# iamgroot42/A-LINK

Hardware: AMD Instinct MI355X
Metric: 112x112 face embeddings/sec (IR-ResNet-100 ArcFace, 512-d, L2-normalised) (higher is better)
Workload: dtype bf16

## Files before the change

a-link_amd/csrc/alink_common.h:

```cpp
#pragma once
#include <hip/hip_runtime.h>
#include <stdint.h>
#include <stddef.h>
#include <string>

#include "../../include/alink_hip.h"
#include "conv_kernel.h"

namespace alink {

void set_error(const char* fmt, ...);
int  hip_fail(hipError_t e, const char* what, const char* file, int line);

#define ALINK_HIP(call)                                                          \
    do {                                                                         \
        hipError_t e__ = (call);                                                 \
        if (e__ != hipSuccess) return ::alink::hip_fail(e__, #call, __FILE__, __LINE__); \
    } while (0)

#define ALINK_REQUIRE(cond, code, ...)          \
    do {                                        \
        if (!(cond)) {                          \
            ::alink::set_error(__VA_ARGS__);    \
            return (code);                      \
// ... 78 lines not shown
    const float* slabs;
    const float* bias;
    float*       out;
    float*       norms;
    int S, M, E;
    float scale;
    int*  nonfinite;
};
hipError_t launch_fc_finish(const FcFinishParams& p, hipStream_t stream);
hipError_t launch_absmax_f16(const void* x, size_t n_elements, unsigned* out_bits, hipStream_t stream);
hipError_t launch_conv_split_finish(int dtype, const ConvParams& p, const float* slabs, int S, hipStream_t stream);

ConvKernel direct_variant(int ksz, int stride, int pad, int H, int W, int Cin, int Cout);
ConvKernel direct_variant_tiles(int ksz, int stride, int pad, int H, int W, int Cin, int Cout);
ConvKernel linear_variant_x2(int ksz, int stride, int pad, int H, int W, int Cin, int Cout);
hipError_t launch_conv(ConvKernel k, int dtype, const ConvParams& p, hipStream_t st);
hipError_t direct_set_attributes();
ConvKernel linear_variant(int ksz, int stride, int pad, int H, int W, int Cin, int Cout);
ConvKernel c64_variant(int ksz, int stride, int pad, int H, int W, int Cin, int Cout);
ConvKernel s2c64_variant(int ksz, int stride, int pad, int H, int W, int Cin, int Cout);
hipError_t launch_conv3x3_linear(ConvKernel k, int dtype, const ConvParams& p, hipStream_t st);
hipError_t launch_conv3x3_c64(int dtype, const ConvParams& p, hipStream_t st);
hipError_t launch_conv3x3_s2c64(int dtype, const ConvParams& p, hipStream_t st);
hipError_t c64_set_attributes();
hipError_t s2c64_set_attributes();
hipError_t linear_set_attributes();
hipError_t linear_check_contract();
bool       front_c64_applies(int dtype, int H, int W, int C0, int Cout);
hipError_t front_c64_set_attributes();
hipError_t launch_front_c64(int dtype, const ConvParams& conv1, const StemParams& stem, void* xs, bool slopes_le_1, hipStream_t st);
bool       unit_c64_applies(int dtype, const ConvParams& c1, const ConvParams& c2);
hipError_t unit_c64_set_attributes();
hipError_t launch_unit_c64(int dtype, const ConvParams& c1, const ConvParams& c2, hipStream_t st);
bool       conv3x3_lat_applies(int dtype, const ConvParams& p);
hipError_t launch_conv3x3_lat(int dtype, const ConvParams& p, hipStream_t stream);
bool       conv_gemm_lat_applies(int dtype, const ConvParams& p);
hipError_t launch_conv_gemm_lat(int dtype, const ConvParams& p, hipStream_t stream);

hipError_t launch_l2norm_bwd(int dtype, const float* g, const float* e, const float* norms, void* dz, int M, int E,
                             hipStream_t st);
hipError_t launch_zero_insert(int dtype, const void* in, void* out, int N, int H, int W, int Ho, int Wo, int C,
                              hipStream_t st);
hipError_t launch_stem_bwd(int dtype, const void* dy0, const void* y0, const float* w, const float* alpha, float* dpix,
                           int N, int H, int W, float mul, int nchw, hipStream_t st);

hipError_t launch_r50_grad_scale(const float* dfeat, int count, int HW, float* scale, hipStream_t st);
hipError_t launch_r50_avgpool_bwd(int dtype, const float* dfeat, const void* y, void* dz, const float* scale, int N, int HW, int C,
                                  hipStream_t st);
hipError_t launch_r50_relu_mask(int dtype, void* g, const void* y, long long count, hipStream_t st);
hipError_t launch_r50_scatter_mask(int dtype, const void* in, const void* y, void* out, int N, int H, int W, int Ho, int Wo, int C,
                                   hipStream_t st);
hipError_t launch_r50_maxpool_bwd(int dtype, const void* y0, const void* pooled, const void* g, void* d0, int N, int H, int W, int C,
                                  int Hp, int Wp, hipStream_t st);
hipError_t launch_r50_stem_bwd(int dtype, const void* d0, const void* wfrag, float* dpix, const float* scale, int N, int H, int W,
                               int Ho, int Wo, int pad_t, int pad_l, int flip, hipStream_t st);
int r50_stem_bwd_max_width();

uint16_t f32_to_bf16_rne(float f);
uint16_t f32_to_f16_rne(float f);

int init_kernels();

__device__ __forceinline__ float relu_keep_nan(float v) { return v < 0.f ? 0.f : v; }
__device__ __forceinline__ float max_keep_nan(float a, float b) { return (a < b || b != b) ? b : a; }

}
// ... 13 lines not shown
```

a-link_amd/csrc/backbone.hip:

```cpp
#include "alink_common.h"

#include <algorithm>
#include <cmath>
#include <cstdarg>
#include <cstdio>
#include <cstring>
#include <map>
#include <string>
#include <vector>

namespace alink {

static thread_local char g_err[1024] = "";
void set_error(const char* fmt, ...) {
    va_list ap;
    va_start(ap, fmt);
    vsnprintf(g_err, sizeof(g_err), fmt, ap);
    va_end(ap);
}
int hip_fail(hipError_t e, const char* what, const char* file, int line) {
    set_error("HIP error %d (%s) in `%s` at %s:%d", (int)e, hipGetErrorString(e), what, file, line);
    return ALINK_EHIP;
}

// ... 660 lines not shown
    if (!traits(k).fine) return 0;
    const int sib = (g_sibling_aware && k != ConvKernel::Linear7) ? siblings : 1;
    return linear_grid(M, Cout, 128) * sib <= g_fine_max ? 1 : 0;
}
int g_ablate = 0;
int g_stop_after = 0;
extern "C" void alink_debug_set_stop_after(int n) { g_stop_after = n; }
int g_stagger = 0;
int g_shard_stagger = 0;
extern "C" void alink_debug_set_shard_stagger(int on) { g_shard_stagger = on; }

int g_fuse_unit = 1;
constexpr int FUSE_UNIT_MIN_N = 64;
extern "C" void alink_debug_set_fuse_unit(int mode) { g_fuse_unit = mode; }
extern "C" void alink_debug_set_stagger(int n) { g_stagger = n < 0 ? 0 : n; }
void* g_stamps = nullptr;
int g_prof_reps = 4;
extern "C" void alink_debug_set_profile_reps(int n) { g_prof_reps = n < 1 ? 1 : n; }
extern "C" void alink_debug_set_ablate(int a) { g_ablate = a; }
extern "C" void alink_debug_set_stamps(void* p) { g_stamps = p; }

static const ConvLayer* fusable_unit(const alink_backbone* bb, const ConvLayer& L, int N, int S, bool cache) {
    if (!g_fuse_unit || (g_fuse_unit == 1 && N < FUSE_UNIT_MIN_N) || cache || S != 1 || g_ablate || g_stamps) return nullptr;
    const int dt = bb->cfg.dtype;
    if (dt != ALINK_DT_BF16 && dt != ALINK_DT_F16) return nullptr;
    const size_t i = (size_t)(&L - bb->convs.data());
    if (L.role != 1 || i + 1 >= bb->convs.size()) return nullptr;
    const ConvLayer& L2 = bb->convs[i + 1];
    if (L2.role != 3 || L2.unit != L.unit || L2.Cin2 || L2.in_buf != L.out_buf || L2.resid_buf != L.in_buf) return nullptr;
    if (L.kernel != ConvKernel::Linear56 || L2.kernel != ConvKernel::Linear56 || L.stride != 1 || L2.stride != 1) return nullptr;
    if (L.Cin != 64 || L.Cout != 64 || L2.Cin != 64 || L2.Cout != 64 || L.Hin != 56 || L.Win != 56) return nullptr;
    if (plan_split(bb, L2, N) != 1) return nullptr;
    return &L2;
}

static int embed_impl(alink_backbone_t* bb, const void* dev_in, int layout, int N, float* dev_out,
                      void* ws, size_t ws_bytes, hipStream_t stream, float* ms, double* flops, int* kind,
                      int* n_launches, const GradLayout* cache = nullptr, int calib = 0, hipEvent_t front_done = nullptr) {
    ALINK_REQUIRE(bb && dev_in && dev_out && ws, ALINK_EINVAL, "NULL argument");
    ALINK_REQUIRE(bb->finalized, ALINK_ESTATE, "alink_embed before alink_backbone_finalize");
    ALINK_REQUIRE(N > 0, ALINK_EINVAL, "n_images must be positive");
    ALINK_REQUIRE(layout >= 0 && layout <= 2, ALINK_EINVAL, "unknown pixel layout %d", layout);
    const alink_ir_cfg& cfg = bb->cfg;
    ALINK_REQUIRE((long long)N * cfg.height * cfg.width * 64 * (cfg.dtype == ALINK_DT_F16X2 ? 2 : 1) < (1ll << 31), ALINK_EINVAL,
                  "batch of %d images exceeds the 2^31-element activation limit; split the batch", N);
    size_t off[7], total;
    ws_layout(bb, N, off, &total);
    if (cache) total = cache->total;
    ALINK_REQUIRE(ws_bytes >= total, ALINK_ENOMEM, "workspace too small: %zu < %zu", ws_bytes, total);
    ALINK_REQUIRE(((uintptr_t)ws & 255) == 0, ALINK_EINVAL, "workspace must be 256-byte aligned");
    char* base = (char*)ws;
    auto buf = [&](int id) -> void* { return base + off[id]; };

    const bool prof = ms != nullptr;
    const int reps = prof ? g_prof_reps : 1;
    const int cap = prof ? *n_launches : 0;
    int nl = 0;
    std::vector<hipEvent_t> ev;
    std::vector<int> split_pairs;
    auto mark = [&]() -> int {
        if (!prof) return ALINK_OK;
        hipEvent_t e;
        ALINK_HIP(hipEventCreate(&e));
        ALINK_HIP(hipEventRecord(e, stream));
        ev.push_back(e);
        return ALINK_OK;
// ... 102 lines not shown
                    ConvParams q = p;
                    if (S > 1) {
                        q.out = buf(6); q.splitk = S; q.ksteps_per_split = p.ksteps_per_split / S;
                    }
                    ALINK_HIP(launch_conv(L.kernel, cfg.dtype, q, stream));
                    if (S > 1) ALINK_HIP(launch_conv_split_finish(cfg.dtype, p, (const float*)buf(6), S, stream));
                }
                return ALINK_OK;
            });
            if (rc) return rc;
            bexp[L.out_buf] = L.e_out;
        } else if (front && &L == &bb->convs[0]) {
            p.stamps = g_stamps;
            for (int r = 0; r < reps; ++r) ALINK_HIP(launch_front_c64(cfg.dtype, p, sp, buf(0), bb->front_slopes_le_1, stream));
            note(conv_flops(p) + 2.0 * N * cfg.height * cfg.width * 64.0 * 27.0, 1);
            if ((rc = mark())) return rc;
            last_out = L.out_buf;
            continue;
        } else if (const ConvLayer* L2 = fusable_unit(bb, L, N, S, cache != nullptr)) {
            ConvParams p2 = p;
            p2.in = buf(L2->in_buf); p2.wgt = L2->d_w; p2.bias = L2->d_bias; p2.alpha = L2->d_alpha;
            p2.resid = buf(L2->resid_buf); p2.out = buf(L2->out_buf);
            p2.Cout = L2->Cout; p2.border_cls = L2->border_cls ? 1 : 0;
            ALINK_REQUIRE(unit_c64_applies(cfg.dtype, p, p2), ALINK_EINVAL, "fused unit %s: launch forms do not apply", L.name.c_str());
            for (int r = 0; r < reps; ++r) ALINK_HIP(launch_unit_c64(cfg.dtype, p, p2, stream));
            note(conv_flops(p), 1);
            if ((rc = mark())) return rc;
            if (prof && nl < cap) split_pairs.push_back(nl - 1);
            note(conv_flops(p2), 1);
            if ((rc = mark())) return rc;
            last_out = L2->out_buf;
            skip_conv2 = true;
            continue;
        } else
        for (int r = 0; r < reps; ++r) {
            ConvParams q = p;
            if (S > 1) {
                q.out = buf(6); q.splitk = S; q.ksteps_per_split = p.ksteps_per_split / S;
            }
            ALINK_HIP(launch_conv(L.kernel, cfg.dtype, q, stream));
            if (S > 1) ALINK_HIP(launch_conv_split_finish(cfg.dtype, p, (const float*)buf(6), S, stream));
        }
        note(conv_flops(p), 1);
        if ((rc = mark())) return rc;
        last_out = L.out_buf;
    }

    {
        ConvParams p{};
        p.in = buf(last_out); p.wgt = bb->d_fc_w; p.bias = nullptr; p.alpha = nullptr; p.resid = nullptr;
        p.out = buf(5); p.zero = bb->d_zero;
        p.N = N; p.H = 1; p.W = 1; p.Cin = bb->fc_K; p.Cout = cfg.emb; p.Ho = 1; p.Wo = 1;
        p.stride = 1; p.ksz = 1; p.pad = 0; p.M = N; p.border_cls = 0;
        p.splitk = bb->fc_splitk; p.ksteps_per_split = bb->fc_kps * (x2 ? 3 : 1);
        p.nprod = (x2 && !calib) ? bb->products : 0;
        ALINK_REQUIRE(p.splitk > 1, ALINK_EINVAL, "FC split-K must be > 1 (K=%d)", bb->fc_K);
        for (int r = 0; r < reps; ++r) ALINK_HIP(launch_conv_igemm(cfg.dtype, p, stream));
        note(conv_flops(p), 2);
        if ((rc = mark())) return rc;
        FcFinishParams f{};
        f.slabs = (const float*)buf(5); f.bias = bb->d_fc_bias; f.out = dev_out;
        f.norms = cache ? (float*)(base + cache->norms) : nullptr;
        f.S = bb->fc_splitk; f.M = N; f.E = cfg.emb;
        f.scale = x2 ? std::ldexp(1.f, -(bexp[last_out] + bb->fc_e_w)) : 1.f;
        f.nonfinite = bb->d_flag;
        for (int r = 0; r < reps; ++r) ALINK_HIP(launch_fc_finish(f, stream));
// ... 398 lines not shown
```

a-link_amd/csrc/conv3x3_direct.hip:

```cpp
#include "conv_device.h"

namespace alink {
namespace {

template <int WPX, int TPW, int TR>
struct Geo {
    static constexpr bool modeA = (TR % WPX) == 0;
    static constexpr bool modeB = !modeA && (TR == TPW);
    static constexpr bool modeC = !modeA && !modeB;
    static_assert(modeA || modeB || (TR == 1), "unsupported tile geometry");
    static constexpr int CPG = modeA ? TR / WPX : 1;
    static constexpr int R = modeA ? TPW / CPG : (modeB ? WPX : TPW * WPX);
    __device__ static constexpr int row(int g, int u) { return modeA ? u / CPG : (modeB ? g : g * TPW + u); }
    __device__ static constexpr int cb(int g, int u)  { return modeA ? g * CPG + u % CPG : (modeB ? u : 0); }
};

template <int A, int B>
struct IC2 { static constexpr int a = A, b = B; };

template <typename T, int WPX, int WCO, int TPW, int TCW, int TR, int PITCH, int NWB, int NWV, bool XDB>
__global__ __launch_bounds__(NWV * 64, 2) void conv3x3_direct_kernel(const ConvParams p) {
    typedef typename Vec8<T>::type vec8;
    typedef Geo<WPX, TPW, TR> G;
    constexpr int NT = NWV * 64;
// ... 277 lines not shown
    }
    return direct_variant_tiles(ksz, stride, pad, H, W, Cin, Cout);
}
ConvKernel direct_variant_tiles(int ksz, int stride, int pad, int H, int W, int Cin, int Cout) {
    if (!g_use_direct || ksz != 3 || stride != 1 || pad != 1 || Cin % 64 || Cout % 64) return ConvKernel::Igemm;
    const ConvKernel lk = linear_variant(ksz, stride, pad, H, W, Cin, Cout);
    if (lk != ConvKernel::Igemm) return lk;
    if (W > 14 * 8 || H < 1) return ConvKernel::Igemm;
    const int tr = (W + 15) / 16, pitch = (W + 2 + 15) / 16 * 16;
    if (g_use_pair) {
        if (tr == 1 && pitch == 16 && W >= 12 && Cout % 128 == 0 && S1::lds_bytes(Cin) <= 80 * 1024) return ConvKernel::PairW14C128;
        if (tr == 2 && pitch == 32 && Cout % 128 == 0 && S3::lds_bytes(Cin) <= 80 * 1024) return ConvKernel::PairW28C128;
    }
    if (tr == 1 && pitch == 16 && W >= 12 && Cout % 256 == 0 && D1::fits(Cin)) return ConvKernel::TileW14C256;
    if (tr == 2 && pitch == 32 && Cout % 256 == 0 && D2::fits(Cin)) return ConvKernel::TileW28C256;
    if (tr == 2 && pitch == 32 && Cout % 128 == 0 && D3::fits(Cin)) return ConvKernel::TileW28C128;
    if (tr == 4 && pitch == 64 && Cout % 128 == 0 && D4::fits(Cin)) return ConvKernel::TileW56C128;
    if (tr == 4 && pitch == 64 && D5::fits(Cin)) return ConvKernel::TileW56C64;
    if (tr == 7 && pitch == 128 && W == 112 && D6::fits(Cin)) return ConvKernel::TileW112C64;
    return ConvKernel::Igemm;
}

hipError_t direct_set_attributes() {
    hipError_t e;
#define A(V)                                                         \
    if ((e = V::set_attr<__bf16>()) != hipSuccess) return e;         \
    if ((e = V::set_attr<_Float16>()) != hipSuccess) return e;
    A(D1) A(D2) A(D3) A(D4) A(D5) A(D6) A(S1) A(S3)
#undef A
    if ((e = c64_set_attributes()) != hipSuccess) return e;
    if ((e = front_c64_set_attributes()) != hipSuccess) return e;
    if ((e = s2c64_set_attributes()) != hipSuccess) return e;
    if ((e = unit_c64_set_attributes()) != hipSuccess) return e;
    return linear_set_attributes();
}

hipError_t launch_conv(ConvKernel k, int dtype, const ConvParams& p, hipStream_t st) {
    if (k == ConvKernel::Igemm) return launch_conv_igemm(dtype, p, st);
    if (k == ConvKernel::Roll112) return launch_conv3x3_c64(dtype, p, st);
    if (k == ConvKernel::Roll112S2) return launch_conv3x3_s2c64(dtype, p, st);
    if (traits(k).channel_block) return launch_conv3x3_linear(k, dtype, p, st);
    if (dtype != ALINK_DT_BF16 && dtype != ALINK_DT_F16) return hipErrorInvalidValue;
    if (p.ksz != 3 || p.stride != 1 || p.pad != 1 || p.splitk != 1) return hipErrorInvalidValue;
    if ((long long)p.N * p.H * p.W * p.Cin >= (1ll << 31)) return hipErrorInvalidValue;
#define L(V) (dtype == ALINK_DT_BF16 ? V::launch<__bf16>(p, st) : V::launch<_Float16>(p, st))
    switch (k) {
        case ConvKernel::TileW14C256: return L(D1);
        case ConvKernel::TileW28C256: return L(D2);
        case ConvKernel::TileW28C128: return L(D3);
        case ConvKernel::TileW56C128: return L(D4);
        case ConvKernel::TileW56C64:  return L(D5);
        case ConvKernel::TileW112C64: return L(D6);
        case ConvKernel::PairW14C128: return L(S1);
        case ConvKernel::PairW28C128: return L(S3);
        default: break;
    }
#undef L
    return hipErrorInvalidValue;
}

}
```

a-link_amd/csrc/conv3x3_s2c64.hip:

```cpp
#include "conv_device.h"

namespace alink {
namespace {

typedef __attribute__((__vector_size__(4 * sizeof(int)))) int i32x4;

constexpr int NT = 256;
constexpr int WI = 112, HI = 112, WO = 56, HO = 56, C = 64;
constexpr int RING = 8;
constexpr int ODDB = (WO + 8 + 1) * 128;
constexpr int EVENB = (WO + 8) * 128;
constexpr int PITCH = ODDB + EVENB;
constexpr int XBYTES = RING * PITCH;
constexpr int KR = 9 * C + C;
constexpr size_t lds_bytes() { return (size_t)XBYTES + C * 4; }

template <typename T, bool SC>
__global__ __launch_bounds__(NT, 1) void conv3x3_s2c64_kernel(const ConvParams p) {
    typedef typename Vec8<T>::type vec8;
    extern __shared__ __attribute__((aligned(16))) char smem[];

    const int tid = threadIdx.x, lane = tid & 63;
    const int wave = __builtin_amdgcn_readfirstlane(tid >> 6);
    const int th = wave >> 1, ch = wave & 1;
    const int q = lane >> 4, lr = lane & 15;

    const T* __restrict__ gin = (const T*)p.in;
    const T* __restrict__ gw = (const T*)p.wgt;
    const T* __restrict__ gz = (const T*)p.zero;

    for (int i = tid; i < RING * 8; i += NT) *(uint4*)(smem + (i >> 3) * PITCH + (i & 7) * 16) = uint4{0u, 0u, 0u, 0u};
    float* const ebias = (float*)(smem + XBYTES);
    for (int i = tid; i < C; i += NT) ebias[i] = p.bias[i];
    const int wpitch = SC ? KR : 9 * C;
    vec8 wr[2][9][2];
#pragma unroll
    for (int ct = 0; ct < 2; ++ct)
#pragma unroll
        for (int tap = 0; tap < 9; ++tap)
#pragma unroll
            for (int ks = 0; ks < 2; ++ks)
                wr[ct][tap][ks] = *(const vec8*)(gw + (size_t)(ch * 32 + 16 * ct + lr) * wpitch + tap * 64 + ks * 32 + 8 * q);
    vec8 ws[2][2];
    if (SC) {
#pragma unroll
        for (int ct = 0; ct < 2; ++ct)
#pragma unroll
            for (int ks = 0; ks < 2; ++ks) ws[ct][ks] = *(const vec8*)(gw + (size_t)(ch * 32 + 16 * ct + lr) * KR + 9 * C + ks * 32 + 8 * q);
    }

    const int d = delta(lr);
    int loff[2][2];
#pragma unroll
    for (int e = 0; e < 2; ++e)
#pragma unroll
        for (int ks = 0; ks < 2; ++ks) loff[e][ks] = (d + e) * 128 + ((((ks << 2) | q) ^ (((d + e) >> 1) & 7)) << 4);

    auto stage_rows = [&](long long in_row0, int r0, int count) __attribute__((always_inline)) {
        for (int j = wave; j < count * 14; j += 4) {
            const int ri = j / 14, jj = j - ri * 14, odd = jj < 7 ? 1 : 0, seg = odd ? jj : jj - 7;
            const int r = r0 + ri, slot = (r + 1) & (RING - 1);
            const int pj = seg * 8 + (lane >> 3);
            const int pos = pj + odd;
            const int piece = (lane & 7) ^ ((pos >> 1) & 7);
            const bool ok = r >= 0;
            const T* src = ok ? gin + ((size_t)(in_row0 + r) * WI + 2 * pj + odd) * C + piece * 8 : gz + (lane & 7) * 8;
            dma16(src, smem + slot * PITCH + (odd ? 0 : ODDB) + (seg * 8 + odd) * 128);
        }
    };
    const T* __restrict__ gx = (const T*)p.in2;
    auto load_sc = [&](long long n, int y, vec8 (&xs)[2][2]) __attribute__((always_inline)) {
#pragma unroll
        for (int t = 0; t < 2; ++t) {
            int x = 16 * (2 * th + t) + d;
            x = x < WO ? x : WO - 1;
            const size_t pix = p.in2_compact ? ((size_t)n * HO + y) * WO + x : ((size_t)n * HI + 2 * y) * WI + 2 * x;
#pragma unroll
            for (int ks = 0; ks < 2; ++ks) xs[t][ks] = *(const vec8*)(gx + pix * C + ks * 32 + 8 * q);
        }
    };
    auto compute = [&](f32x4 (&acc)[2][2], int y, const vec8 (&xs)[2][2]) __attribute__((always_inline)) {
#pragma unroll
        for (int ct = 0; ct < 2; ++ct)
#pragma unroll
            for (int t = 0; t < 2; ++t) acc[ct][t] = f32x4{0.f, 0.f, 0.f, 0.f};
        int sb[3];
#pragma unroll
        for (int ky = 0; ky < 3; ++ky) sb[ky] = ((2 * y + ky) & (RING - 1)) * PITCH + 2 * th * 2048;
        auto frag = [&](int st, int t) __attribute__((always_inline)) -> vec8 {
            const int tap = st >> 1, ks = st & 1, ky = tap / 3, kx = tap % 3;
            return *(const vec8*)(smem + sb[ky] + loff[kx == 2 ? 1 : 0][ks] + (kx == 1 ? ODDB : 0) + 2048 * t);
        };
        vec8 pf[2][2];
#pragma unroll
        for (int t = 0; t < 2; ++t) pf[0][t] = frag(0, t);
#pragma unroll
        for (int st = 0; st < 18; ++st) {
            if (st + 1 < 18) {
#pragma unroll
                for (int t = 0; t < 2; ++t) pf[(st + 1) & 1][t] = frag(st + 1, t);
            }
            const int tap = st >> 1, ks = st & 1;
#pragma unroll
            for (int ct = 0; ct < 2; ++ct)
#pragma unroll
                for (int t = 0; t < 2; ++t) acc[ct][t] = mfma16<T>(wr[ct][tap][ks], pf[st & 1][t], acc[ct][t]);
        }
        if (SC) {
#pragma unroll
            for (int ks = 0; ks < 2; ++ks)
#pragma unroll
                for (int ct = 0; ct < 2; ++ct)
#pragma unroll
                    for (int t = 0; t < 2; ++t) acc[ct][t] = mfma16<T>(ws[ct][ks], xs[t][ks], acc[ct][t]);
        }
    };
    auto epilogue = [&](const f32x4 (&acc)[2][2], long long n, int y) __attribute__((always_inline)) {
        const f32x4 b0 = *(const f32x4*)(ebias + ch * 32 + 8 * q), b1 = *(const f32x4*)(ebias + ch * 32 + 8 * q + 4);
#pragma unroll
        for (int t = 0; t < 2; ++t) {
            const int x = 16 * (2 * th + t) + d;
            const bool live = x < WO;
            const size_t el = (((size_t)n * HO + y) * WO + (live ? x : 0)) * C + ch * 32 + 8 * q;
            float v[8];
#pragma unroll
            for (int j = 0; j < 4; ++j) { v[j] = acc[0][t][j] + b0[j]; v[4 + j] = acc[1][t][j] + b1[j]; }
            if (!SC && p.alpha) {
#pragma unroll
                for (int i = 0; i < 8; ++i) v[i] = v[i] > 0.f ? v[i] : v[i] * p.alpha[ch * 32 + 8 * q + i];
            }
            if (!SC && p.resid) {
                const vec8 r8 = *(const vec8*)((const T*)p.resid + el);
#pragma unroll
                for (int i = 0; i < 8; ++i) v[i] += (float)r8[i];
            }
            vec8 o8;
#pragma unroll
            for (int i = 0; i < 8; ++i) o8[i] = (T)v[i];
            if (live) *(vec8*)((T*)p.out + el) = o8;
        }
    };
    auto top_of_pass = [&](bool staged, bool loaded, bool stored) __attribute__((always_inline)) {
        const int n = (staged ? 7 : 0) + (loaded ? 4 : 0) + (stored ? 2 : 0);
        switch (n) {
            case 13: wait_then_barrier<13>(); break;
            case 11: wait_then_barrier<11>(); break;
            case 9:  wait_then_barrier<9>(); break;
            case 7:  wait_then_barrier<7>(); break;
            case 6:  wait_then_barrier<6>(); break;
            case 4:  wait_then_barrier<4>(); break;
            case 2:  wait_then_barrier<2>(); break;
            default: wait_then_barrier<0>(); break;
        }
    };

    const long long nrows = (long long)p.N * HO;
    const long long r0 = nrows * blockIdx.x / gridDim.x, r1 = nrows * (blockIdx.x + 1) / gridDim.x;
    for (long long rr = r0; rr < r1;) {
        const long long n = rr / HO;
        const int y0 = (int)(rr - n * HO);
        int np = HO - y0;
        if (np > r1 - rr) np = (int)(r1 - rr);
        rr += np;
        const long long in_row0 = n * HI;
        wait_then_barrier<0>();
        stage_rows(in_row0, 2 * y0 - 1, 3);
        if (np > 1) stage_rows(in_row0, 2 * y0 + 2, 2);
        vec8 xsA[2][2], xsB[2][2];
        if (SC) load_sc(n, y0, xsA);
        f32x4 acc[2][2];
#pragma unroll 1
        for (int k = 0; k < np; k += 2) {
            if (k == 0) { if (np > 1) wait_then_barrier<7 + (SC ? 4 : 0)>(); else wait_then_barrier<SC ? 4 : 0>(); }
            else        top_of_pass(k + 1 < np, SC && k < np, true);
            if (k + 2 < np) stage_rows(in_row0, 2 * (y0 + k + 2), 2);
            if (SC && k + 1 < np) load_sc(n, y0 + k + 1, xsB);
            compute(acc, y0 + k, xsA);
            epilogue(acc, n, y0 + k);
            if (k + 1 < np) {
                top_of_pass(k + 2 < np, SC && k + 1 < np, true);
                if (k + 3 < np) stage_rows(in_row0, 2 * (y0 + k + 3), 2);
                if (SC && k + 2 < np) load_sc(n, y0 + k + 2, xsA);
                compute(acc, y0 + k + 1, xsB);
                epilogue(acc, n, y0 + k + 1);
            }
        }
    }
}

bool g_use_s2c64 = true;

}

extern "C" void alink_debug_set_s2direct(int on) { g_use_s2c64 = on != 0; }

ConvKernel s2c64_variant(int ksz, int stride, int pad, int H, int W, int Cin, int Cout) {
    if (!g_use_s2c64 || ksz != 3 || stride != 2 || pad != 1 || Cin != C || Cout != C || H != HI || W != WI) return ConvKernel::Igemm;
    return ConvKernel::Roll112S2;
}

hipError_t s2c64_set_attributes() {
    hipError_t e;
#define A(T, SC) if ((e = hipFuncSetAttribute((const void*)conv3x3_s2c64_kernel<T, SC>, hipFuncAttributeMaxDynamicSharedMemorySize, (int)lds_bytes())) != hipSuccess) return e;
    A(__bf16, true) A(__bf16, false) A(_Float16, true) A(_Float16, false)
#undef A
    return hipSuccess;
}

hipError_t launch_conv3x3_s2c64(int dtype, const ConvParams& p, hipStream_t st) {
    if (p.ksz != 3 || p.stride != 2 || p.pad != 1 || p.Cin != C || p.Cout != C || p.H != HI || p.W != WI) return hipErrorInvalidValue;
    if (p.splitk != 1 || p.dact || p.post_relu || p.border_cls || p.N <= 0) return hipErrorInvalidValue;
    if (p.in2 && (p.Cin2 != C || p.alpha || p.resid)) return hipErrorInvalidValue;
    if ((long long)p.N * HI * WI * C >= (1ll << 31)) return hipErrorInvalidValue;
    if (dtype != ALINK_DT_BF16 && dtype != ALINK_DT_F16) return hipErrorInvalidValue;
    const long long nrows = (long long)p.N * HO;
    const unsigned grid = (unsigned)(nrows < 256 ? nrows : 256);
    if (dtype == ALINK_DT_BF16) {
        if (p.in2) hipLaunchKernelGGL((conv3x3_s2c64_kernel<__bf16, true>), dim3(grid), dim3(NT), lds_bytes(), st, p);
        else       hipLaunchKernelGGL((conv3x3_s2c64_kernel<__bf16, false>), dim3(grid), dim3(NT), lds_bytes(), st, p);
    } else {
        if (p.in2) hipLaunchKernelGGL((conv3x3_s2c64_kernel<_Float16, true>), dim3(grid), dim3(NT), lds_bytes(), st, p);
        else       hipLaunchKernelGGL((conv3x3_s2c64_kernel<_Float16, false>), dim3(grid), dim3(NT), lds_bytes(), st, p);
    }
    return hipGetLastError();
}

}
```

include/alink_hip_debug.h:

```cpp
#ifndef ALINK_HIP_DEBUG_H
#define ALINK_HIP_DEBUG_H

#include <stddef.h>

#ifdef __cplusplus
extern "C" {
#endif

void alink_debug_set_linear(int mode);
void alink_debug_set_generic_epilogue(int on);
void alink_debug_set_direct(int on);
void alink_debug_set_pair(int on);
void alink_debug_set_c64(int on);
void alink_debug_set_s2direct(int on);
void alink_debug_set_fuse_stem(int on);
void alink_debug_set_fuse_unit(int mode);
void alink_debug_set_fuse_shortcut(int on);
void alink_debug_set_dma(int on);
void alink_debug_set_fine_max(int n);
void alink_debug_set_sibling_aware(int on);
void alink_debug_set_latency_form(int max_pixels);
void alink_debug_set_latency_tiles(int form);
void alink_debug_set_stagger(int n);
void alink_debug_set_shard_stagger(int on);

void alink_debug_set_tiny_step(int on);
void alink_debug_set_mini_step(int on);
void alink_debug_set_head_bf16_mfma(int on);

void alink_debug_set_smallres_overlap(int on);
void alink_debug_set_smallres_one_update(int on);

void alink_debug_set_stop_after(int n);
void alink_debug_set_profile_reps(int n);
void alink_debug_set_ablate(int a);
void alink_debug_set_stamps(void* dev_u64);
int alink_debug_lds_oob_probe(float* dev_out516, void* stream);
int alink_debug_linear_contract_ok(void);


struct alink_resnet50;
struct alink_backbone;
int alink_debug_resnet50_grad_cache_info(const struct alink_resnet50* r, int n_images, int index, size_t* byte_offset, int* H,
                                         int* W, int* C, char* name_buf, int name_len);
int alink_debug_backbone_grad_cache_info(const struct alink_backbone* bb, int n_images, int index, size_t* byte_offset, int* H,
                                         int* W, int* C, char* name_buf, int name_len);

#ifdef __cplusplus
}
// ... 3 lines not shown
```

Measured before the change: 44940.

## Add dedicated 64-to-128 channel 3x3 conv kernel for 56x56 stage opener

```diff
diff --git a/a-link_amd/csrc/alink_common.h b/a-link_amd/csrc/alink_common.h
--- a/a-link_amd/csrc/alink_common.h
+++ b/a-link_amd/csrc/alink_common.h
@@ -134,6 +134,9 @@
 bool       unit_c64_applies(int dtype, const ConvParams& c1, const ConvParams& c2);
 hipError_t unit_c64_set_attributes();
 hipError_t launch_unit_c64(int dtype, const ConvParams& c1, const ConvParams& c2, hipStream_t st);
+bool       open_c64_applies(int dtype, const ConvParams& c);
+hipError_t open_c64_set_attributes();
+hipError_t launch_open_c64(int dtype, const ConvParams& c, hipStream_t st);
 bool       conv3x3_lat_applies(int dtype, const ConvParams& p);
 hipError_t launch_conv3x3_lat(int dtype, const ConvParams& p, hipStream_t stream);
 bool       conv_gemm_lat_applies(int dtype, const ConvParams& p);
diff --git a/a-link_amd/csrc/backbone.hip b/a-link_amd/csrc/backbone.hip
--- a/a-link_amd/csrc/backbone.hip
+++ b/a-link_amd/csrc/backbone.hip
@@ -716,6 +716,17 @@
     if (L.Cin != 64 || L.Cout != 64 || L2.Cin != 64 || L2.Cout != 64 || L.Hin != 56 || L.Win != 56) return nullptr;
     if (plan_split(bb, L2, N) != 1) return nullptr;
     return &L2;
+}
+
+int g_open_c64 = 1;
+constexpr int OPEN_C64_MIN_N = 64;
+extern "C" void alink_debug_set_open_c64(int mode) { g_open_c64 = mode; }
+static bool open_c64_layer(const alink_backbone* bb, const ConvLayer& L, int N, int S, bool cache) {
+    if (!g_open_c64 || (g_open_c64 == 1 && N < OPEN_C64_MIN_N) || cache || S != 1 || g_ablate || g_stamps) return false;
+    const int dt = bb->cfg.dtype;
+    if (dt != ALINK_DT_BF16 && dt != ALINK_DT_F16) return false;
+    return L.role == 1 && L.kernel == ConvKernel::Linear56 && L.stride == 1 && L.Cin == 64 && L.Cout == 128 && L.Hin == 56 &&
+           L.Win == 56 && !L.Cin2 && L.resid_buf < 0;
 }
 
 static int embed_impl(alink_backbone_t* bb, const void* dev_in, int layout, int N, float* dev_out,
@@ -884,6 +895,8 @@
             last_out = L2->out_buf;
             skip_conv2 = true;
             continue;
+        } else if (open_c64_layer(bb, L, N, S, cache != nullptr) && open_c64_applies(cfg.dtype, p)) {
+            for (int r = 0; r < reps; ++r) ALINK_HIP(launch_open_c64(cfg.dtype, p, stream));
         } else
         for (int r = 0; r < reps; ++r) {
             ConvParams q = p;
diff --git a/a-link_amd/csrc/conv3x3_direct.hip b/a-link_amd/csrc/conv3x3_direct.hip
--- a/a-link_amd/csrc/conv3x3_direct.hip
+++ b/a-link_amd/csrc/conv3x3_direct.hip
@@ -333,6 +333,7 @@
     if ((e = front_c64_set_attributes()) != hipSuccess) return e;
     if ((e = s2c64_set_attributes()) != hipSuccess) return e;
     if ((e = unit_c64_set_attributes()) != hipSuccess) return e;
+    if ((e = open_c64_set_attributes()) != hipSuccess) return e;
     return linear_set_attributes();
 }
 
diff --git a/a-link_amd/csrc/conv3x3_s2c64.hip b/a-link_amd/csrc/conv3x3_s2c64.hip
--- a/a-link_amd/csrc/conv3x3_s2c64.hip
+++ b/a-link_amd/csrc/conv3x3_s2c64.hip
@@ -7,17 +7,24 @@
 
 constexpr int NT = 256;
 constexpr int WI = 112, HI = 112, WO = 56, HO = 56, C = 64;
-constexpr int RING = 8;
-constexpr int ODDB = (WO + 8 + 1) * 128;
-constexpr int EVENB = (WO + 8) * 128;
-constexpr int PITCH = ODDB + EVENB;
-constexpr int XBYTES = RING * PITCH;
+template <int R>
+struct Ring {
+    static constexpr int ODDB = (R == 8 ? WO + 8 + 1 : WO + 1) * 128;
+    static constexpr int EVENB = (WO + 8) * 128;
+    static constexpr int PITCH = ODDB + EVENB;
+    static constexpr int XBYTES = R * PITCH;
+    static constexpr size_t lds_bytes() { return (size_t)XBYTES + C * 4; }
+    static constexpr int slot(int r) { return R == 8 ? (r & 7) : r % R; }
+};
+static_assert(Ring<8>::lds_bytes() == 132352, "the 8-slot form as it was");
+static_assert(Ring<5>::lds_bytes() <= 80 * 1024 && Ring<5>::lds_bytes() <= 160 * 1024 - 74768,
+              "two per CU, and one beside a 28-wide tile workgroup");
 constexpr int KR = 9 * C + C;
-constexpr size_t lds_bytes() { return (size_t)XBYTES + C * 4; }
-
-template <typename T, bool SC>
-__global__ __launch_bounds__(NT, 1) void conv3x3_s2c64_kernel(const ConvParams p) {
+
+template <typename T, bool SC, int R>
+__global__ __launch_bounds__(NT, R == 5 ? 2 : 1) void conv3x3_s2c64_kernel(const ConvParams p) {
     typedef typename Vec8<T>::type vec8;
+    constexpr int RING = R, ODDB = Ring<R>::ODDB, PITCH = Ring<R>::PITCH, XBYTES = Ring<R>::XBYTES;
     extern __shared__ __attribute__((aligned(16))) char smem[];
 
     const int tid = threadIdx.x, lane = tid & 63;
@@ -59,7 +66,7 @@
     auto stage_rows = [&](long long in_row0, int r0, int count) __attribute__((always_inline)) {
         for (int j = wave; j < count * 14; j += 4) {
             const int ri = j / 14, jj = j - ri * 14, odd = jj < 7 ? 1 : 0, seg = odd ? jj : jj - 7;
-            const int r = r0 + ri, slot = (r + 1) & (RING - 1);
+            const int r = r0 + ri, slot = Ring<R>::slot(r + 1);
             const int pj = seg * 8 + (lane >> 3);
             const int pos = pj + odd;
             const int piece = (lane & 7) ^ ((pos >> 1) & 7);
@@ -86,7 +93,7 @@
             for (int t = 0; t < 2; ++t) acc[ct][t] = f32x4{0.f, 0.f, 0.f, 0.f};
         int sb[3];
 #pragma unroll
-        for (int ky = 0; ky < 3; ++ky) sb[ky] = ((2 * y + ky) & (RING - 1)) * PITCH + 2 * th * 2048;
+        for (int ky = 0; ky < 3; ++ky) sb[ky] = Ring<R>::slot(2 * y + ky) * PITCH + 2 * th * 2048;
         auto frag = [&](int st, int t) __attribute__((always_inline)) -> vec8 {
             const int tap = st >> 1, ks = st & 1, ky = tap / 3, kx = tap % 3;
             return *(const vec8*)(smem + sb[ky] + loff[kx == 2 ? 1 : 0][ks] + (kx == 1 ? ODDB : 0) + 2048 * t);
@@ -164,35 +171,63 @@
         rr += np;
         const long long in_row0 = n * HI;
         wait_then_barrier<0>();
-        stage_rows(in_row0, 2 * y0 - 1, 3);
-        if (np > 1) stage_rows(in_row0, 2 * y0 + 2, 2);
-        vec8 xsA[2][2], xsB[2][2];
-        if (SC) load_sc(n, y0, xsA);
-        f32x4 acc[2][2];
+        if constexpr (R == 5) {
+            stage_rows(in_row0, 2 * y0 - 1, 3);
+            asm volatile("" ::: "memory");
+            vec8 xsA[2][2], xsB[2][2];
+            if (SC) load_sc(n, y0, xsA);
+            f32x4 acc[2][2];
 #pragma unroll 1
-        for (int k = 0; k < np; k += 2) {
-            if (k == 0) { if (np > 1) wait_then_barrier<7 + (SC ? 4 : 0)>(); else wait_then_barrier<SC ? 4 : 0>(); }
-            else        top_of_pass(k + 1 < np, SC && k < np, true);
-            if (k + 2 < np) stage_rows(in_row0, 2 * (y0 + k + 2), 2);
-            if (SC && k + 1 < np) load_sc(n, y0 + k + 1, xsB);
-            compute(acc, y0 + k, xsA);
-            epilogue(acc, n, y0 + k);
-            if (k + 1 < np) {
-                top_of_pass(k + 2 < np, SC && k + 1 < np, true);
-                if (k + 3 < np) stage_rows(in_row0, 2 * (y0 + k + 3), 2);
-                if (SC && k + 2 < np) load_sc(n, y0 + k + 2, xsA);
-                compute(acc, y0 + k + 1, xsB);
-                epilogue(acc, n, y0 + k + 1);
+            for (int k = 0; k < np; k += 2) {
+                if (k == 0) wait_then_barrier<SC ? 4 : 0>();
+                else        wait_then_barrier<SC ? 6 : 2>();
+                if (k + 1 < np) stage_rows(in_row0, 2 * (y0 + k + 1), 2);
+                asm volatile("" ::: "memory");
+                if (SC && k + 1 < np) load_sc(n, y0 + k + 1, xsB);
+                compute(acc, y0 + k, xsA);
+                epilogue(acc, n, y0 + k);
+                if (k + 1 < np) {
+                    wait_then_barrier<SC ? 6 : 2>();
+                    if (k + 2 < np) stage_rows(in_row0, 2 * (y0 + k + 2), 2);
+                    asm volatile("" ::: "memory");
+                    if (SC && k + 2 < np) load_sc(n, y0 + k + 2, xsA);
+                    compute(acc, y0 + k + 1, xsB);
+                    epilogue(acc, n, y0 + k + 1);
+                }
+            }
+        } else {
+            stage_rows(in_row0, 2 * y0 - 1, 3);
+            if (np > 1) stage_rows(in_row0, 2 * y0 + 2, 2);
+            vec8 xsA[2][2], xsB[2][2];
+            if (SC) load_sc(n, y0, xsA);
+            f32x4 acc[2][2];
+    #pragma unroll 1
+            for (int k = 0; k < np; k += 2) {
+                if (k == 0) { if (np > 1) wait_then_barrier<7 + (SC ? 4 : 0)>(); else wait_then_barrier<SC ? 4 : 0>(); }
+                else        top_of_pass(k + 1 < np, SC && k < np, true);
+                if (k + 2 < np) stage_rows(in_row0, 2 * (y0 + k + 2), 2);
+                if (SC && k + 1 < np) load_sc(n, y0 + k + 1, xsB);
+                compute(acc, y0 + k, xsA);
+                epilogue(acc, n, y0 + k);
+                if (k + 1 < np) {
+                    top_of_pass(k + 2 < np, SC && k + 1 < np, true);
+                    if (k + 3 < np) stage_rows(in_row0, 2 * (y0 + k + 3), 2);
+                    if (SC && k + 2 < np) load_sc(n, y0 + k + 2, xsA);
+                    compute(acc, y0 + k + 1, xsB);
+                    epilogue(acc, n, y0 + k + 1);
+                }
             }
         }
     }
 }
 
 bool g_use_s2c64 = true;
+int g_s2c64_slots = 8;
 
 }
 
 extern "C" void alink_debug_set_s2direct(int on) { g_use_s2c64 = on != 0; }
+extern "C" void alink_debug_set_s2c64_form(int slots) { g_s2c64_slots = slots == 5 ? 5 : 8; }
 
 ConvKernel s2c64_variant(int ksz, int stride, int pad, int H, int W, int Cin, int Cout) {
     if (!g_use_s2c64 || ksz != 3 || stride != 2 || pad != 1 || Cin != C || Cout != C || H != HI || W != WI) return ConvKernel::Igemm;
@@ -201,8 +236,9 @@
 
 hipError_t s2c64_set_attributes() {
     hipError_t e;
-#define A(T, SC) if ((e = hipFuncSetAttribute((const void*)conv3x3_s2c64_kernel<T, SC>, hipFuncAttributeMaxDynamicSharedMemorySize, (int)lds_bytes())) != hipSuccess) return e;
-    A(__bf16, true) A(__bf16, false) A(_Float16, true) A(_Float16, false)
+#define A(T, SC, R) if ((e = hipFuncSetAttribute((const void*)conv3x3_s2c64_kernel<T, SC, R>, hipFuncAttributeMaxDynamicSharedMemorySize, (int)Ring<R>::lds_bytes())) != hipSuccess) return e;
+    A(__bf16, true, 8) A(__bf16, false, 8) A(_Float16, true, 8) A(_Float16, false, 8)
+    A(__bf16, true, 5) A(__bf16, false, 5) A(_Float16, true, 5) A(_Float16, false, 5)
 #undef A
     return hipSuccess;
 }
@@ -214,14 +250,22 @@
     if ((long long)p.N * HI * WI * C >= (1ll << 31)) return hipErrorInvalidValue;
     if (dtype != ALINK_DT_BF16 && dtype != ALINK_DT_F16) return hipErrorInvalidValue;
     const long long nrows = (long long)p.N * HO;
-    const unsigned grid = (unsigned)(nrows < 256 ? nrows : 256);
+    const int slots = g_s2c64_slots;
+    const long long cap = slots == 5 ? 512 : 256;
+    const unsigned grid = (unsigned)(nrows < cap ? nrows : cap);
+#define L(T, SC)                                                                                                                    \
+    do {                                                                                                                            \
+        if (slots == 5) hipLaunchKernelGGL((conv3x3_s2c64_kernel<T, SC, 5>), dim3(grid), dim3(NT), Ring<5>::lds_bytes(), st, p);    \
+        else            hipLaunchKernelGGL((conv3x3_s2c64_kernel<T, SC, 8>), dim3(grid), dim3(NT), Ring<8>::lds_bytes(), st, p);    \
+    } while (0)
     if (dtype == ALINK_DT_BF16) {
-        if (p.in2) hipLaunchKernelGGL((conv3x3_s2c64_kernel<__bf16, true>), dim3(grid), dim3(NT), lds_bytes(), st, p);
-        else       hipLaunchKernelGGL((conv3x3_s2c64_kernel<__bf16, false>), dim3(grid), dim3(NT), lds_bytes(), st, p);
+        if (p.in2) L(__bf16, true);
+        else       L(__bf16, false);
     } else {
-        if (p.in2) hipLaunchKernelGGL((conv3x3_s2c64_kernel<_Float16, true>), dim3(grid), dim3(NT), lds_bytes(), st, p);
-        else       hipLaunchKernelGGL((conv3x3_s2c64_kernel<_Float16, false>), dim3(grid), dim3(NT), lds_bytes(), st, p);
+        if (p.in2) L(_Float16, true);
+        else       L(_Float16, false);
     }
+#undef L
     return hipGetLastError();
 }
 
diff --git a/a-link_amd/csrc/open_c64.hip b/a-link_amd/csrc/open_c64.hip
--- /dev/null
+++ b/a-link_amd/csrc/open_c64.hip
@@ -0,0 +1,203 @@
+#include "conv_device.h"
+
+namespace alink {
+namespace {
+
+constexpr int W = 56;
+constexpr int CO = 128;
+constexpr int NT = 512;
+constexpr int ROWB = W * 128;
+constexpr int XR = 8;
+constexpr int TBL = (9 * CO + CO) * 4;
+constexpr int XOFF = TBL;
+constexpr size_t LDS_BYTES = (size_t)XOFF + XR * ROWB;
+static_assert(TBL % 1024 == 0 && TBL >= 256, "row slots stay 1 KB aligned and a tap at column -1 stays at a positive address");
+
+struct OpenParams {
+    const void*  x;
+    const void*  w;
+    const float* b;
+    const float* a;
+    void*        out;
+    const void*  zero;
+    int N;
+};
+
+template <typename T, int HALF>
+__device__ __forceinline__ void open_wave(const OpenParams& p, char* smem, int g, int wave, long long r0, int npairs) {
+    typedef typename Vec8<T>::type vec8;
+    constexpr int NTL = HALF == 0 ? 4 : 3;
+    constexpr int U0 = HALF == 0 ? 0 : 4;
+    const int lane = threadIdx.x & 63;
+    const int q = lane >> 4, lr = lane & 15;
+    const int d = delta(lr);
+    const long long nrows = (long long)p.N * W;
+
+    const T* __restrict__ gw = (const T*)p.w;
+    vec8 wr[2][9][2];
+#pragma unroll
+    for (int ct = 0; ct < 2; ++ct)
+#pragma unroll
+        for (int tap = 0; tap < 9; ++tap)
+#pragma unroll
+            for (int ks = 0; ks < 2; ++ks)
+                wr[ct][tap][ks] = *(const vec8*)(gw + (size_t)(g * 32 + 16 * ct + lr) * 576 + tap * 64 + ks * 32 + 8 * q);
+
+    int lo[3][2];
+#pragma unroll
+    for (int kx = 0; kx < 3; ++kx)
+#pragma unroll
+        for (int ks = 0; ks < 2; ++ks) {
+            const int pos = d + kx - 1;
+            const int v = pos * 128 + ((((ks << 2) | q) ^ ((pos >> 1) & 7)) << 4);
+            lo[kx][ks] = HALF == 0 ? v : (v ^ 64);
+        }
+    const bool sel3 = HALF == 0 && d >= 8;
+    const int x64 = sel3 ? 64 : 0;
+    unsigned bcode = 0;
+#pragma unroll
+    for (int u = 0; u < NTL; ++u) {
+        const int P = 16 * (U0 + u) + d, r = P >= W ? 1 : 0, c = P - W * r;
+        bcode |= ((r ? 2u : 1u) | (c == 0 ? 4u : 0u) | (c == W - 1 ? 8u : 0u)) << (4 * u);
+    }
+
+    const float* const eb = (const float*)smem;
+    const float* const ea = eb + 9 * CO;
+    const T* __restrict__ gx = (const T*)p.x;
+    const T* __restrict__ gz = (const T*)p.zero;
+
+    auto stage_pair = [&](int j) {
+        for (int uidx = wave; uidx < 14; uidx += 8) {
+            const int ri = uidx / 7, seg = uidx - ri * 7;
+            const long long row = r0 - 1 + 2 * j + ri;
+            const int slot = (2 * j + ri) % XR;
+            const int px = seg * 8 + (lane >> 3);
+            const int piece = (lane & 7) ^ ((px >> 1) & 7);
+            const bool ok = row >= 0 && row < nrows;
+            const T* src = ok ? gx + (size_t)row * (W * 64) + (unsigned)(px * 64 + piece * 8) : gz + (lane & 7) * 8;
+            dma16(src, smem + XOFF + slot * ROWB + seg * 1024);
+        }
+    };
+    stage_pair(0), stage_pair(1);
+
+#pragma unroll 1
+    for (int k = 0; k < npairs; ++k) {
+        if (k == 0) wait_then_barrier<0>();
+        else        wait_then_barrier<NTL>();
+        if (k + 1 < npairs) stage_pair(k + 2);
+        const long long ya = r0 + 2 * k;
+        int sb[4];
+#pragma unroll
+        for (int i = 0; i < 4; ++i) sb[i] = XOFF + ((2 * k + i) % XR) * ROWB;
+        const int m0 = (int)(ya % W), m1 = m0 + 1;
+        const unsigned topm = m0 == 0 ? 1u : 0u;
+        const unsigned botm = m1 == W - 1 ? 2u : 0u;
+
+        f32x4 acc[2][NTL];
+#pragma unroll
+        for (int ct = 0; ct < 2; ++ct)
+#pragma unroll
+            for (int u = 0; u < NTL; ++u) acc[ct][u] = f32x4{0.f, 0.f, 0.f, 0.f};
+        auto fetch = [&](vec8 (&pf)[NTL], int st) {
+            const int tap = st >> 1, ks = st & 1, ky = tap / 3, kx = tap % 3;
+            const unsigned tb = (ky == 0 ? topm : (ky == 2 ? botm : 0u)) | (kx == 0 ? 4u : 0u) | (kx == 2 ? 8u : 0u);
+            unsigned bnow = bcode;
+            asm volatile("" : "+v"(bnow));
+            const int blo = sb[ky], bhi = sb[ky + 1] - ROWB;
+#pragma unroll
+            for (int u = 0; u < NTL; ++u) {
+                const unsigned t = bnow & (tb << (4 * u));
+                const int far = (int)(t << (18 - 4 * u));
+                int a;
+                if (HALF == 1)      a = bhi + lo[kx][ks] + 2048 * (U0 + u);
+                else if (u < 3)     a = blo + lo[kx][ks] + 2048 * u;
+                else                a = (sel3 ? bhi : blo) + (lo[kx][ks] ^ x64) + 2048 * 3;
+                pf[u] = *(const vec8*)(smem + (a + far));
+            }
+        };
+        vec8 pf[2][NTL];
+        fetch(pf[0], 0);
+#pragma unroll
+        for (int st = 0; st < 18; ++st) {
+            if (st + 1 < 18) fetch(pf[(st + 1) & 1], st + 1);
+            const int tap = st >> 1, ks = st & 1;
+#pragma unroll
+            for (int ct = 0; ct < 2; ++ct)
+#pragma unroll
+                for (int u = 0; u < NTL; ++u) acc[ct][u] = mfma16<T>(wr[ct][tap][ks], pf[st & 1][u], acc[ct][u]);
+        }
+
+        T* const orow = (T*)p.out + (size_t)ya * (W * CO) + g * 32;
+        int de = d;
+        asm volatile("" : "+v"(de));
+        const f32x4 a0 = *(const f32x4*)(ea + g * 32 + 8 * q), a1 = *(const f32x4*)(ea + g * 32 + 8 * q + 4);
+#pragma unroll
+        for (int u = 0; u < NTL; ++u) {
+            const int P = 16 * (U0 + u) + de, r = P >= W ? 1 : 0, c = P - W * r;
+            const int m = r ? m1 : m0;
+            const int cls = (m == 0 ? 0 : (m == W - 1 ? 2 : 1)) * 3 + (c == 0 ? 0 : (c == W - 1 ? 2 : 1));
+            const f32x4 b0 = *(const f32x4*)(eb + cls * CO + g * 32 + 8 * q);
+            const f32x4 b1 = *(const f32x4*)(eb + cls * CO + g * 32 + 8 * q + 4);
+            float v[8];
+#pragma unroll
+            for (int j = 0; j < 4; ++j) { v[j] = acc[0][u][j] + b0[j]; v[4 + j] = acc[1][u][j] + b1[j]; }
+#pragma unroll
+            for (int j = 0; j < 4; ++j) {
+                v[j] = v[j] > 0.f ? v[j] : v[j] * a0[j];
+                v[4 + j] = v[4 + j] > 0.f ? v[4 + j] : v[4 + j] * a1[j];
+            }
+            vec8 o8;
+#pragma unroll
+            for (int i = 0; i < 8; ++i) o8[i] = (T)v[i];
+            *(vec8*)(orow + (unsigned)(P * CO + 8 * q)) = o8;
+        }
+    }
+}
+
+template <typename T>
+__global__ __launch_bounds__(NT, 1) void open_c64_kernel(const OpenParams p) {
+    extern __shared__ __attribute__((aligned(16))) char smem[];
+    const int tid = threadIdx.x;
+    {
+        float* const eb = (float*)smem;
+        for (int i = tid; i < 9 * CO + CO; i += NT) eb[i] = i < 9 * CO ? p.b[i] : p.a[i - 9 * CO];
+    }
+    const long long pairs = (long long)p.N * (W / 2);
+    const int nwg = gridDim.x;
+    const int lid = xcd_remap(blockIdx.x, nwg);
+    const long long p0 = pairs * lid / nwg, p1 = pairs * (lid + 1) / nwg;
+    const long long r0 = 2 * p0;
+    const int npairs = (int)(p1 - p0);
+    const int wave = __builtin_amdgcn_readfirstlane(tid >> 6);
+    if (wave < 4) open_wave<T, 0>(p, smem, wave & 3, wave, r0, npairs);
+    else          open_wave<T, 1>(p, smem, wave & 3, wave, r0, npairs);
+}
+
+}
+
+hipError_t open_c64_set_attributes() {
+    hipError_t e = hipFuncSetAttribute((const void*)open_c64_kernel<__bf16>, hipFuncAttributeMaxDynamicSharedMemorySize, (int)LDS_BYTES);
+    if (e == hipSuccess)
+        e = hipFuncSetAttribute((const void*)open_c64_kernel<_Float16>, hipFuncAttributeMaxDynamicSharedMemorySize, (int)LDS_BYTES);
+    return e;
+}
+
+bool open_c64_applies(int dtype, const ConvParams& c) {
+    if (dtype != ALINK_DT_BF16 && dtype != ALINK_DT_F16) return false;
+    return c.ksz == 3 && c.stride == 1 && c.pad == 1 && c.H == W && c.W == W && c.Cin == 64 && c.Cout == CO && c.splitk == 1 &&
+           !c.dact && !c.post_relu && !c.in2 && !c.ablate && !c.stamps && c.N > 0 && c.alpha && c.border_cls && !c.resid &&
+           (long long)c.N * W * W * CO < (1ll << 31);
+}
+
+hipError_t launch_open_c64(int dtype, const ConvParams& c, hipStream_t st) {
+    if (!open_c64_applies(dtype, c)) return hipErrorInvalidValue;
+    OpenParams p{};
+    p.x = c.in; p.w = c.wgt; p.b = c.bias; p.a = c.alpha; p.out = c.out; p.zero = c.zero; p.N = c.N;
+    const long long pairs = (long long)p.N * (W / 2);
+    const unsigned grid = (unsigned)(pairs < 256 ? pairs : 256);
+    if (dtype == ALINK_DT_BF16) hipLaunchKernelGGL(open_c64_kernel<__bf16>, dim3(grid), dim3(NT), LDS_BYTES, st, p);
+    else                        hipLaunchKernelGGL(open_c64_kernel<_Float16>, dim3(grid), dim3(NT), LDS_BYTES, st, p);
+    return hipGetLastError();
+}
+
+}
diff --git a/include/alink_hip_debug.h b/include/alink_hip_debug.h
--- a/include/alink_hip_debug.h
+++ b/include/alink_hip_debug.h
@@ -13,8 +13,10 @@
 void alink_debug_set_pair(int on);
 void alink_debug_set_c64(int on);
 void alink_debug_set_s2direct(int on);
+void alink_debug_set_s2c64_form(int slots);
 void alink_debug_set_fuse_stem(int on);
 void alink_debug_set_fuse_unit(int mode);
+void alink_debug_set_open_c64(int mode);
 void alink_debug_set_fuse_shortcut(int on);
 void alink_debug_set_dma(int on);
 void alink_debug_set_fine_max(int n);
```

Measured after the change: 45160, median of 6. No clear change (+0.5%).

## Double wave count in s2c64 conv to compute two output rows per block pass

Applied to the files above, without the earlier changes.

```diff
diff --git a/a-link_amd/csrc/conv3x3_s2c64.hip b/a-link_amd/csrc/conv3x3_s2c64.hip
--- a/a-link_amd/csrc/conv3x3_s2c64.hip
+++ b/a-link_amd/csrc/conv3x3_s2c64.hip
@@ -5,9 +5,9 @@
 
 typedef __attribute__((__vector_size__(4 * sizeof(int)))) int i32x4;
 
-constexpr int NT = 256;
+constexpr int NT = 512;
 constexpr int WI = 112, HI = 112, WO = 56, HO = 56, C = 64;
-constexpr int RING = 8;
+constexpr int RING = 9;
 constexpr int ODDB = (WO + 8 + 1) * 128;
 constexpr int EVENB = (WO + 8) * 128;
 constexpr int PITCH = ODDB + EVENB;
@@ -22,7 +22,8 @@
 
     const int tid = threadIdx.x, lane = tid & 63;
     const int wave = __builtin_amdgcn_readfirstlane(tid >> 6);
-    const int th = wave >> 1, ch = wave & 1;
+    const int g = wave >> 2;
+    const int th = (wave >> 1) & 1, ch = wave & 1;
     const int q = lane >> 4, lr = lane & 15;
 
     const T* __restrict__ gin = (const T*)p.in;
@@ -56,16 +57,19 @@
 #pragma unroll
         for (int ks = 0; ks < 2; ++ks) loff[e][ks] = (d + e) * 128 + ((((ks << 2) | q) ^ (((d + e) >> 1) & 7)) << 4);
 
-    auto stage_rows = [&](long long in_row0, int r0, int count) __attribute__((always_inline)) {
-        for (int j = wave; j < count * 14; j += 4) {
-            const int ri = j / 14, jj = j - ri * 14, odd = jj < 7 ? 1 : 0, seg = odd ? jj : jj - 7;
-            const int r = r0 + ri, slot = (r + 1) & (RING - 1);
-            const int pj = seg * 8 + (lane >> 3);
-            const int pos = pj + odd;
-            const int piece = (lane & 7) ^ ((pos >> 1) & 7);
-            const bool ok = r >= 0;
-            const T* src = ok ? gin + ((size_t)(in_row0 + r) * WI + 2 * pj + odd) * C + piece * 8 : gz + (lane & 7) * 8;
-            dma16(src, smem + slot * PITCH + (odd ? 0 : ODDB) + (seg * 8 + odd) * 128);
+    const int odd = wave & 1;
+    unsigned lvo[2];
+#pragma unroll
+    for (int sp = 0; sp < 2; ++sp) lvo[sp] = 2 * (lane >> 3) * C + (((lane & 7) ^ ((4 * sp + (((lane >> 3) + odd) >> 1)) & 7)) << 3);
+    auto stage_plane = [&](long long in_row0, int r, int slot, bool top) __attribute__((always_inline)) {
+        char* const dst = smem + slot * PITCH + (odd ? 128 : ODDB);
+        if (top && r < 0) {
+#pragma unroll
+            for (int seg = 0; seg < 7; ++seg) dma16(gz + (lane & 7) * 8, dst + seg * 1024);
+        } else {
+            const T* src = gin + ((size_t)(in_row0 + r) * WI + odd) * C;
+#pragma unroll
+            for (int seg = 0; seg < 7; ++seg) dma16(src + seg * 16 * C + lvo[seg & 1], dst + seg * 1024);
         }
     };
     const T* __restrict__ gx = (const T*)p.in2;
@@ -79,14 +83,14 @@
             for (int ks = 0; ks < 2; ++ks) xs[t][ks] = *(const vec8*)(gx + pix * C + ks * 32 + 8 * q);
         }
     };
-    auto compute = [&](f32x4 (&acc)[2][2], int y, const vec8 (&xs)[2][2]) __attribute__((always_inline)) {
+    auto compute = [&](f32x4 (&acc)[2][2], int s, const vec8 (&xs)[2][2]) __attribute__((always_inline)) {
 #pragma unroll
         for (int ct = 0; ct < 2; ++ct)
 #pragma unroll
             for (int t = 0; t < 2; ++t) acc[ct][t] = f32x4{0.f, 0.f, 0.f, 0.f};
         int sb[3];
 #pragma unroll
-        for (int ky = 0; ky < 3; ++ky) sb[ky] = ((2 * y + ky) & (RING - 1)) * PITCH + 2 * th * 2048;
+        for (int ky = 0; ky < 3; ++ky) sb[ky] = (s + ky < RING ? s + ky : s + ky - RING) * PITCH + 2 * th * 2048;
         auto frag = [&](int st, int t) __attribute__((always_inline)) -> vec8 {
             const int tap = st >> 1, ks = st & 1, ky = tap / 3, kx = tap % 3;
             return *(const vec8*)(smem + sb[ky] + loff[kx == 2 ? 1 : 0][ks] + (kx == 1 ? ODDB : 0) + 2048 * t);
@@ -140,59 +144,45 @@
             if (live) *(vec8*)((T*)p.out + el) = o8;
         }
     };
-    auto top_of_pass = [&](bool staged, bool loaded, bool stored) __attribute__((always_inline)) {
-        const int n = (staged ? 7 : 0) + (loaded ? 4 : 0) + (stored ? 2 : 0);
-        switch (n) {
-            case 13: wait_then_barrier<13>(); break;
-            case 11: wait_then_barrier<11>(); break;
-            case 9:  wait_then_barrier<9>(); break;
-            case 7:  wait_then_barrier<7>(); break;
-            case 6:  wait_then_barrier<6>(); break;
-            case 4:  wait_then_barrier<4>(); break;
-            case 2:  wait_then_barrier<2>(); break;
-            default: wait_then_barrier<0>(); break;
-        }
-    };
-
-    const long long nrows = (long long)p.N * HO;
-    const long long r0 = nrows * blockIdx.x / gridDim.x, r1 = nrows * (blockIdx.x + 1) / gridDim.x;
-    for (long long rr = r0; rr < r1;) {
-        const long long n = rr / HO;
-        const int y0 = (int)(rr - n * HO);
-        int np = HO - y0;
-        if (np > r1 - rr) np = (int)(r1 - rr);
-        rr += np;
+    __builtin_amdgcn_s_waitcnt(0x0F70);
+    const long long npairs = (long long)p.N * (HO / 2);
+    const long long p0 = npairs * blockIdx.x / gridDim.x, p1 = npairs * (blockIdx.x + 1) / gridDim.x;
+    for (long long pp = p0; pp < p1;) {
+        const long long n = pp / (HO / 2);
+        const int y0 = 2 * (int)(pp - n * (HO / 2));
+        int np = (HO - y0) / 2;
+        if (np > p1 - pp) np = (int)(p1 - pp);
+        pp += np;
         const long long in_row0 = n * HI;
         wait_then_barrier<0>();
-        stage_rows(in_row0, 2 * y0 - 1, 3);
-        if (np > 1) stage_rows(in_row0, 2 * y0 + 2, 2);
-        vec8 xsA[2][2], xsB[2][2];
-        if (SC) load_sc(n, y0, xsA);
+        for (int job = wave; job < 2 * 5; job += 8) stage_plane(in_row0, 2 * y0 - 1 + (job >> 1), job >> 1, true);
+        int s0 = 0;
         f32x4 acc[2][2];
+        vec8 xs[2][2];
 #pragma unroll 1
-        for (int k = 0; k < np; k += 2) {
-            if (k == 0) { if (np > 1) wait_then_barrier<7 + (SC ? 4 : 0)>(); else wait_then_barrier<SC ? 4 : 0>(); }
-            else        top_of_pass(k + 1 < np, SC && k < np, true);
-            if (k + 2 < np) stage_rows(in_row0, 2 * (y0 + k + 2), 2);
-            if (SC && k + 1 < np) load_sc(n, y0 + k + 1, xsB);
-            compute(acc, y0 + k, xsA);
-            epilogue(acc, n, y0 + k);
+        for (int k = 0; k < np; ++k) {
+            const int y = y0 + 2 * k;
+            if (k == 0) wait_then_barrier<0>();
+            else        wait_then_barrier<2>();
+            if (SC) load_sc(n, y + g, xs);
             if (k + 1 < np) {
-                top_of_pass(k + 2 < np, SC && k + 1 < np, true);
-                if (k + 3 < np) stage_rows(in_row0, 2 * (y0 + k + 3), 2);
-                if (SC && k + 2 < np) load_sc(n, y0 + k + 2, xsA);
-                compute(acc, y0 + k + 1, xsB);
-                epilogue(acc, n, y0 + k + 1);
-            }
+                const int sn = s0 + 5 + (wave >> 1);
+                stage_plane(in_row0, 2 * y + 4 + (wave >> 1), sn < RING ? sn : sn - RING, false);
+            }
+            compute(acc, s0 + 2 * g, xs);
+            epilogue(acc, n, y + g);
+            s0 = s0 + 4 < RING ? s0 + 4 : s0 + 4 - RING;
         }
     }
 }
 
 bool g_use_s2c64 = true;
+int g_s2c64_grid = 0;
 
 }
 
 extern "C" void alink_debug_set_s2direct(int on) { g_use_s2c64 = on != 0; }
+extern "C" void alink_debug_set_s2c64_grid(int n) { g_s2c64_grid = n > 0 ? n : 0; }
 
 ConvKernel s2c64_variant(int ksz, int stride, int pad, int H, int W, int Cin, int Cout) {
     if (!g_use_s2c64 || ksz != 3 || stride != 2 || pad != 1 || Cin != C || Cout != C || H != HI || W != WI) return ConvKernel::Igemm;
@@ -213,8 +203,9 @@
     if (p.in2 && (p.Cin2 != C || p.alpha || p.resid)) return hipErrorInvalidValue;
     if ((long long)p.N * HI * WI * C >= (1ll << 31)) return hipErrorInvalidValue;
     if (dtype != ALINK_DT_BF16 && dtype != ALINK_DT_F16) return hipErrorInvalidValue;
-    const long long nrows = (long long)p.N * HO;
-    const unsigned grid = (unsigned)(nrows < 256 ? nrows : 256);
+    const long long npairs = (long long)p.N * (HO / 2);
+    unsigned grid = (unsigned)(npairs < 256 ? npairs : 256);
+    if (g_s2c64_grid > 0 && grid > (unsigned)g_s2c64_grid) grid = (unsigned)g_s2c64_grid;
     if (dtype == ALINK_DT_BF16) {
         if (p.in2) hipLaunchKernelGGL((conv3x3_s2c64_kernel<__bf16, true>), dim3(grid), dim3(NT), lds_bytes(), st, p);
         else       hipLaunchKernelGGL((conv3x3_s2c64_kernel<__bf16, false>), dim3(grid), dim3(NT), lds_bytes(), st, p);
diff --git a/include/alink_hip_debug.h b/include/alink_hip_debug.h
--- a/include/alink_hip_debug.h
+++ b/include/alink_hip_debug.h
@@ -13,6 +13,7 @@
 void alink_debug_set_pair(int on);
 void alink_debug_set_c64(int on);
 void alink_debug_set_s2direct(int on);
+void alink_debug_set_s2c64_grid(int n);
 void alink_debug_set_fuse_stem(int on);
 void alink_debug_set_fuse_unit(int mode);
 void alink_debug_set_fuse_shortcut(int on);
```

Measured after the change: 47690 before, 47890 after, median of 6. About the same (+0.4%).
